# ablab/spades

Hardware: NVIDIA H100
Metric: Mk-mers/s (extract+count+index) k=55, 150 bp reads (higher is better)
Workload: dtype u64

## Files before the change

spades_b200/csrc/count.cu:

```cuda
#include <time.h>

#include <algorithm>

#include "sgpu_internal.h"

namespace sg {

__device__ __forceinline__ void prefetch_l2(const void *p) { asm volatile("prefetch.global.L2 [%0];" ::"l"(p)); }

struct ReadsSrc {
    const uint64_t *words;
    const uint64_t *offs;
    const uint32_t *lens;
    int64_t n;
    uint64_t nwords;
    int K;
    static constexpr int kIds = 24;
    static constexpr int kIdLines = 48;
    static constexpr bool kSubRanges = true;
    __device__ __forceinline__ uint64_t first_word(int64_t item) const { return offs[item]; }
    __device__ __forceinline__ uint32_t len(int64_t item) const { return lens[item]; }
    __device__ __forceinline__ void prefetch_items(int64_t item, int lane) const {
        if (lane == 0) prefetch_l2(lens + item);
        else if (lane == 1 && item + 16 < n) prefetch_l2(offs + item + 16);
// ... 172 lines not shown
    const int lane = threadIdx.x & 31;
    const int64_t item = t * kRollTile + lane;
    uint32_t s = 0;
    if (item < src.n) {
        const int L = (int)src.len(item);
        const uint32_t w = L >= src.K ? (uint32_t)(L - src.K + 1) : 0u;
        s = (w + kRollWin<BOTH> - 1) / kRollWin<BOTH>;
    }
    for (int o = 16; o; o >>= 1) s += __shfl_down_sync(0xffffffffu, s, o);
    if (lane == 0) out[t] = s * Src::kIds;
}

struct RollUnit { int it, j0, cnt; };
template <bool BOTH>
__device__ __forceinline__ RollUnit roll_unit(const RollWarp &rw, int nitems, uint32_t u, uint32_t unif, int K) {
    constexpr int C = kRollWin<BOTH>;
    RollUnit q;
    q.it = find_item_u(rw.pref, nitems, u, unif);
    q.j0 = (int)(u - rw.pref[q.it]) * C;
    const int nwin = (int)rw.len[q.it] - K + 1;
    q.cnt = nwin - q.j0 < C ? nwin - q.j0 : C;
    return q;
}

template <int NW, class Src, bool BOTH>
__global__ void __launch_bounds__(kRollThreads, 2) levelA_count_roll_k(Src src, LevelA p, uint32_t *__restrict__ blk_counts,
                                                                      const uint64_t *__restrict__ tile_off, uint16_t *__restrict__ ids) {
    extern __shared__ __align__(16) unsigned char sm_raw[];
    uint32_t *hist = reinterpret_cast<uint32_t *>(sm_raw);
    RollWarp &rw = *roll_warp_slice(sm_raw, p.PA);
    for (uint32_t i = threadIdx.x; i < p.PA; i += blockDim.x) hist[i] = 0;
    __syncthreads();
    const int K = p.K;
    const int lane = threadIdx.x & 31, warp = threadIdx.x >> 5;
    const int64_t ntiles = (src.n + kRollTile - 1) / kRollTile;
    const int64_t per = (ntiles + gridDim.x - 1) / gridDim.x;
    const int64_t t0 = (int64_t)blockIdx.x * per, t1 = min(ntiles, t0 + per);
    for (int64_t t = t0 + warp; t < t1; t += kRollWarps) {
        const int64_t item0 = t * kRollTile;
        const int nitems = (int)min((int64_t)kRollTile, src.n - item0);
        uint32_t unif = 0;
        bool staged = false;
        const bool has_next = t + kRollWarps < t1;
        const int64_t nx = (t + kRollWarps) * kRollTile;
        uint64_t next_w0 = 0;
        if (has_next) {
            next_w0 = src.first_word(nx);
            src.prefetch_items(nx, lane);
        }
        const uint32_t nunits = roll_warp_setup<BOTH>(src, item0, nitems, rw, &unif, &staged);
        uint64_t *row = ids ? reinterpret_cast<uint64_t *>(ids + tile_off[t]) : nullptr;
        for (uint32_t u = lane; u < nunits; u += 32) {
            const RollUnit q = roll_unit<BOTH>(rw, nitems, u, unif, K);
            const uint64_t *seq = staged ? static_cast<const uint64_t *>(rw.words + rw.off[q.it]) : src.words + src.first_word(item0 + q.it);
            RollState<NW> st;
            roll_init<NW>(st, seq, q.j0, K, q.cnt);
            const int nrec = BOTH ? 2 * q.cnt : q.cnt;
#pragma unroll 1
            for (int g = 0; g < Src::kIds / 4; ++g) {
                uint64_t acc = 0;
#pragma unroll
                for (int e = 0; e < 4; ++e) {
                    const int s = 4 * g + e;
                    uint32_t id = 0xffffu;
                    if (s < nrec) {
                        if (s > 0 && !(BOTH && (e & 1))) roll_next<NW>(st, K);
                        const Kmer<NW> k = BOTH ? ((e & 1) ? st.r : st.f) : kmer_is_minimal<NW>(st.f, st.r) ? st.f : st.r;
                        uint32_t part;
                        if (part_of<NW>(p, k, &part)) { atomicAdd(&hist[part], 1u); id = part; }
                    }
                    acc |= (uint64_t)id << (16 * e);
                }
                if (row) row[(size_t)u * (Src::kIds / 4) + g] = acc;
            }
        }
        if (has_next && lane < 10 && next_w0 + 16 * lane < src.nwords) prefetch_l2(src.words + next_w0 + 16 * lane);
        __syncwarp();
    }
    __syncthreads();
    uint32_t *out = blk_counts + (size_t)blockIdx.x * p.PA;
    for (uint32_t i = threadIdx.x; i < p.PA; i += blockDim.x) out[i] += hist[i];
}

static const uint32_t kABatchNoTag = 0xffffffffu;
static const int kABatchPartBits = 13;
static const uint32_t kABatchMin = 1024;
template <int NW> struct ABatch {
    static constexpr size_t rec_bytes() { return NW * sizeof(uint64_t) + sizeof(uint32_t) + sizeof(uint16_t); }
};
__host__ __device__ __forceinline__ size_t abatch_offset(uint32_t PA) {
    return ((((size_t)2 * PA * 4 + 15) & ~(size_t)15) + (size_t)kRollWarps * sizeof(RollWarp) + 15) & ~(size_t)15;
}

template <int NW, class Src, bool BOTH, bool HAS_IDS>
__global__ void __launch_bounds__(kRollThreads, 2) levelA_scatter_roll_k(Src src, LevelA p, uint64_t *__restrict__ base, uint64_t *__restrict__ out,
                                                                        const uint64_t *__restrict__ tile_off, const uint16_t *__restrict__ ids,
                                                                        uint32_t id_lo, uint32_t row_stride, uint32_t q_lo, uint64_t ids_len, uint32_t cap) {
    extern __shared__ __align__(16) unsigned char sm_raw[];
    __shared__ uint32_t s_fill;
    __shared__ uint32_t warp_tot[kRollWarps];
    const uint32_t PA = p.PA;
    uint32_t *cur = reinterpret_cast<uint32_t *>(sm_raw);
    uint32_t *cnt = cur + PA;
    RollWarp &rw = *roll_warp_slice(sm_raw, 2 * PA);
    uint64_t *stage = reinterpret_cast<uint64_t *>(sm_raw + abatch_offset(PA));
    uint32_t *tags = reinterpret_cast<uint32_t *>(stage + (size_t)cap * NW);
    uint16_t *idx = reinterpret_cast<uint16_t *>(tags + cap);
    uint64_t *mybase = base + (size_t)blockIdx.x * row_stride + q_lo;
    const uint64_t region0 = mybase[0];
    for (uint32_t i = threadIdx.x; i < PA; i += blockDim.x) { cur[i] = (uint32_t)(mybase[i] - region0); cnt[i] = 0; }
    if (threadIdx.x == 0) s_fill = 0;
    __syncthreads();
    uint64_t *const out0 = out + region0 * NW;
    const int K = p.K;
    const int lane = threadIdx.x & 31, warp = threadIdx.x >> 5;
    const uint32_t lt_mask = (1u << lane) - 1u;
    const int64_t ntiles = (src.n + kRollTile - 1) / kRollTile;
    const int64_t per = (ntiles + gridDim.x - 1) / gridDim.x;
    const int64_t t0 = (int64_t)blockIdx.x * per, t1 = min(ntiles, t0 + per);

    int64_t t = t0 + warp;
    bool need_setup = true;
    int nitems = 0;
    uint32_t nunits = 0, unif = 0;
    bool staged = false;
    uint64_t next_w0 = 0, next_row = 0;
    const ulonglong2 *row = nullptr;
    int u = 0, s = 0, cnt_w = 0;
    RollState<NW> st;
    uint64_t idq[Src::kIds / 4];
    for (;;) {
        while (t < t1) {
            if (need_setup) {
                const int64_t item0 = t * kRollTile;
                nitems = (int)min((int64_t)kRollTile, src.n - item0);
                const int64_t nx = (t + kRollWarps) * kRollTile;
                if (t + kRollWarps < t1) {
                    next_w0 = src.first_word(nx);
                    src.prefetch_items(nx, lane);
                    if (HAS_IDS) next_row = tile_off[t + kRollWarps];
                }
                nunits = roll_warp_setup<BOTH>(src, item0, nitems, rw, &unif, &staged);
                if (HAS_IDS) row = reinterpret_cast<const ulonglong2 *>(ids + tile_off[t]);
                u = lane - 32; s = cnt_w = 0;
                need_setup = false;
            }
            if (s >= cnt_w && u < (int)nunits) {
                u += 32;
                if (u < (int)nunits) {
                    if (HAS_IDS) {
#pragma unroll
                        for (int v = 0; v < Src::kIds / 8; ++v) {
                            const ulonglong2 x = __ldg(row + (size_t)u * (Src::kIds / 8) + v);
                            idq[2 * v] = x.x; idq[2 * v + 1] = x.y;
                        }
                    }
                    const RollUnit q = roll_unit<BOTH>(rw, nitems, (uint32_t)u, unif, K);
                    const uint64_t *seq = staged ? static_cast<const uint64_t *>(rw.words + rw.off[q.it]) : src.words + src.first_word(t * kRollTile + q.it);
                    roll_init<NW>(st, seq, q.j0, K, q.cnt);
                    s = 0; cnt_w = BOTH ? 2 * q.cnt : q.cnt;
                }
            }
            const bool act = s < cnt_w;
            if (!__any_sync(0xffffffffu, act)) {
                if (t + kRollWarps < t1) {
                    if (lane < 10 && next_w0 + 16 * lane < src.nwords) prefetch_l2(src.words + next_w0 + 16 * lane);
                    if (HAS_IDS) {
                        if ((Src::kIdLines >= 32 || lane < Src::kIdLines) && next_row + 64 * lane < ids_len) prefetch_l2(ids + next_row + 64 * lane);
                        if (lane < Src::kIdLines - 32 && next_row + 64 * (32 + lane) < ids_len) prefetch_l2(ids + next_row + 64 * (32 + lane));
                    }
                }
                __syncwarp();
                t += kRollWarps;
                need_setup = true;
                continue;
            }
            uint32_t part = 0;
            bool mine = false;
            Kmer<NW> k;
            if (act) {
                if (HAS_IDS) {
                    part = (uint32_t)(idq[0] & 0xffffu) - id_lo;
                    mine = part < PA;
                }
                if (!HAS_IDS || mine) {
                    const bool fwd = BOTH ? !(s & 1) : kmer_is_minimal<NW>(st.f, st.r);
#pragma unroll
                    for (int j = 0; j < NW; ++j) k.w[j] = fwd ? st.f.w[j] : st.r.w[j];
                }
                if (!HAS_IDS) mine = part_of<NW>(p, k, &part);
            }
            const uint32_t bal = __ballot_sync(0xffffffffu, mine);
            if (bal) {
                const uint32_t n = __popc(bal);
                uint32_t b0 = 0;
                if (lane == 0) b0 = atomicAdd(&s_fill, n);
                b0 = __shfl_sync(0xffffffffu, b0, 0);
                if (b0 + n > cap) {
                    if (b0 < cap && (uint32_t)lane < cap - b0) tags[b0 + lane] = kABatchNoTag;
                    break;
                }
                if (mine) {
                    const uint32_t i = b0 + __popc(bal & lt_mask);
                    const uint32_t rank = atomicAdd(&cnt[part], 1u) & 0xffffu;
                    store_rec<NW>(stage + (size_t)i * NW, k);
                    tags[i] = (rank << kABatchPartBits) | part;
                }
            }
            if (act && ++s < cnt_w) {
                if (!BOTH || !(s & 1)) roll_next<NW>(st, K);
                if (HAS_IDS) {
                    if ((s & 3) == 0) {
#pragma unroll
                        for (int v = 0; v + 1 < Src::kIds / 4; ++v) idq[v] = idq[v + 1];
                    } else {
                        idq[0] >>= 16;
                    }
                }
            }
        }
        const bool more = __syncthreads_or(t < t1);
        const uint32_t nslots = min(s_fill, cap);
        const uint32_t own = (PA + kRollThreads - 1) / kRollThreads;
        const uint32_t j0 = min(PA, threadIdx.x * own), j1 = min(PA, j0 + own);
        uint32_t sum = 0;
        for (uint32_t j = j0; j < j1; ++j) sum += cnt[j] & 0xffffu;
        uint32_t inc = sum;
#pragma unroll
        for (int o = 1; o < 32; o <<= 1) {
            const uint32_t v = __shfl_up_sync(0xffffffffu, inc, o);
            if (lane >= o) inc += v;
        }
        if (lane == 31) warp_tot[warp] = inc;
        __syncthreads();
        uint32_t wb = 0, total = 0;
#pragma unroll
        for (int w = 0; w < kRollWarps; ++w) { const uint32_t v = warp_tot[w]; if (w < warp) wb += v; total += v; }
        uint32_t o = wb + inc - sum;
        for (uint32_t j = j0; j < j1; ++j) {
            const uint32_t c = cnt[j] & 0xffffu;
            o += c;
            cnt[j] = o << 16;
            cur[j] += c;
        }
        if (threadIdx.x == 0) s_fill = 0;
        __syncthreads();
        for (uint32_t i = threadIdx.x; i < nslots; i += kRollThreads) {
            const uint32_t tg = tags[i];
            if (tg == kABatchNoTag) continue;
            idx[(cnt[tg & ((1u << kABatchPartBits) - 1)] >> 16) - 1 - (tg >> kABatchPartBits)] = (uint16_t)i;
        }
        __syncthreads();
        for (uint32_t q = threadIdx.x; q < total; q += kRollThreads) {
            const uint32_t i = idx[q], tg = tags[i];
            const uint32_t slot = cur[tg & ((1u << kABatchPartBits) - 1)] - 1 - (tg >> kABatchPartBits);
            store_rec_stream<NW>(out0 + (size_t)slot * NW, load_rec<NW>(stage + (size_t)i * NW));
        }
        __syncthreads();
        if (!more) break;
    }
    for (uint32_t i = threadIdx.x; i < PA; i += blockDim.x) mybase[i] = region0 + cur[i];
}

struct Seg {
    uint64_t start;
    uint64_t len;
    uint32_t bits;
    uint32_t bb;
};

__global__ void seg_init_k(const uint64_t *__restrict__ part_start, const uint64_t *__restrict__ part_total, uint32_t PA, int rA,
                           uint32_t b_lo, Seg *__restrict__ segs) {
    uint32_t part = blockIdx.x * blockDim.x + threadIdx.x;
    if (part >= PA) return;
    Seg s;
    s.start = part_start[part]; s.len = part_total[part]; s.bits = (uint32_t)rA; s.bb = ((b_lo + (part >> rA)) << 1) | 0u;
    segs[part] = s;
}

struct Pieces {
    const uint64_t *pbase;
    const uint32_t *cnt;
    uint32_t cnt_stride, PA;
    int G;
};
static const int kMaxPieces = 1024;

__global__ void stage_rows_k(const uint32_t *__restrict__ cnt, uint32_t cnt_stride, uint32_t PA, uint64_t *__restrict__ rel, uint64_t *__restrict__ row_total) {
    __shared__ uint64_t wsum[8];
    __shared__ uint64_t carry_s;
    const uint32_t *row = cnt + (size_t)blockIdx.x * cnt_stride;
    uint64_t *out = rel + (size_t)blockIdx.x * PA;
    const int lane = threadIdx.x & 31, warp = threadIdx.x >> 5;
    if (threadIdx.x == 0) carry_s = 0;
    __syncthreads();
    for (uint32_t b = 0; b < PA; b += blockDim.x) {
        const uint32_t i = b + threadIdx.x;
        const uint64_t v = i < PA ? row[i] : 0;
        uint64_t inc = v;
#pragma unroll
        for (int o = 1; o < 32; o <<= 1) {
            uint64_t t = __shfl_up_sync(0xffffffffu, inc, o);
            if (lane >= o) inc += t;
        }
        if (lane == 31) wsum[warp] = inc;
        __syncthreads();
        uint64_t wb = 0, all = 0;
        for (int w = 0; w < 8; ++w) { if (w < warp) wb += wsum[w]; all += wsum[w]; }
        const uint64_t carry = carry_s;
        if (i < PA) out[i] = carry + wb + inc - v;
        __syncthreads();
        if (threadIdx.x == 0) carry_s = carry + all;
        __syncthreads();
    }
    if (threadIdx.x == 0) row_total[blockIdx.x] = carry_s;
}
__global__ void stage_add_k(uint64_t *__restrict__ rel, const uint64_t *__restrict__ row_start, uint32_t PA, int G) {
    const uint64_t i = (uint64_t)blockIdx.x * blockDim.x + threadIdx.x;
    if (i >= (uint64_t)G * PA) return;
    rel[i] += row_start[i / PA];
}

struct RefinePlan { uint32_t cap, target, rmax; int total_bits; };
__device__ __forceinline__ int plan_r(const RefinePlan &rp, uint64_t len, uint32_t bits) {
    if (len <= rp.cap) return 0;
    int rem = rp.total_bits - (int)bits;
    if (rem <= 0) return 0;
    uint64_t want = (len + rp.target - 1) / rp.target;
    int r = 1;
    while (r < (int)rp.rmax && (1ull << r) < want) ++r;
    return r < rem ? r : rem;
}
__global__ void refine_plan_k(const Seg *__restrict__ segs, uint64_t n, RefinePlan rp, uint32_t *__restrict__ nchild, uint32_t *__restrict__ isw, int force_all) {
    uint64_t i = (uint64_t)blockIdx.x * blockDim.x + threadIdx.x;
    if (i >= n) return;
    int r = plan_r(rp, segs[i].len, segs[i].bits);
    nchild[i] = r ? (1u << r) : 1u;
    isw[i] = (r || force_all) ? 1u : 0u;
}
__global__ void refine_copy_k(const Seg *__restrict__ segs, uint64_t n, const uint32_t *__restrict__ isw, const uint64_t *__restrict__ child_base,
                              const uint64_t *__restrict__ work_pos, Seg *__restrict__ nsegs, uint64_t *__restrict__ worklist) {
// ... 622 lines not shown
            refine_k<NW, false><<<grid, kRThreads, sm, st>>>(segs.p, worklist.p, tot[1], cbase.p, rp, K, X.p, Y.p, nsegs_arr.p, wcounter.p, Pieces());
        }
        ctx->launches++;
        SG_CUDA(cudaGetLastError());
        tr.mark("refine round");
        (round == 0 ? ctx->times.refine_splits_round0 : ctx->times.refine_splits_later) += tot[0] - nsegs;
        ++rounds;
        segs = std::move(nsegs_arr);
        nsegs = tot[0];
    }
    ctx->times.refine_rounds_max = std::max(ctx->times.refine_rounds_max, rounds);
    ctx->times.refine += tm.stop();
    DArr<uint32_t> ndist(ctx, nsegs + 1);
    DArr<unsigned long long> stats(ctx, 4);
    SG_CUDA(cudaMemsetAsync(ndist.p, 0, ndist.bytes(), st));
    SG_CUDA(cudaMemsetAsync(stats.p, 0, 32, st));
    SG_CUDA(cudaMemsetAsync(wcounter.p, 0, 8, st));
    tm.start();
    {
        auto launch = [&](auto kernel, size_t smem) {
            SG_CUDA(cudaFuncSetAttribute(kernel, cudaFuncAttributeMaxDynamicSharedMemorySize, (int)smem));
            int occ = 1;
            SG_CUDA(cudaOccupancyMaxActiveBlocksPerMultiprocessor(&occ, kernel, kSThreads, smem));
            if (occ < 1) occ = 1;
            int grid = (int)std::min<uint64_t>(nsegs, (uint64_t)ctx->num_sms * occ);
            if (grid < 1) grid = 1;
            kernel<<<grid, kSThreads, smem, st>>>(segs.p, nsegs, K, X.p, Y.p, ndist.p, wcounter.p, stats.p);
        };
        constexpr int bins = 1 << kSortBinBits;
        launch(local_sort3_k<NW, kSortBinBits, CAP>, (size_t)(CAP + kResCap) * NW * sizeof(uint64_t) + (size_t)3 * bins * sizeof(uint32_t) +
                                                         ((size_t)2 * bins + 2 + kResCap) * sizeof(uint16_t) + 16);
        ctx->launches++;
        SG_CUDA(cudaGetLastError());
    }
    DArr<uint64_t> dbase(ctx, nsegs + 1);
    exclusive_scan_u32_to_u64(ctx, ndist.p, dbase.p, nsegs + 1);
    uint64_t D = 0;
    unsigned long long h_stats[4];
    SG_CUDA(cudaMemcpyAsync(&D, dbase.p + nsegs, 8, cudaMemcpyDeviceToHost, st));
    SG_CUDA(cudaMemcpyAsync(h_stats, stats.p, 32, cudaMemcpyDeviceToHost, st));
    SG_CUDA(cudaStreamSynchronize(st));
    ctx->times.local_sort += tm.stop();
    tr.mark("local sort");
    SG_CHECK(h_stats[0] == 0, 6, "internal: oversize segment with unfixed key bits reached the local sort");
    ctx->times.sort_lsd_fallbacks += h_stats[1];
    ctx->times.sort_oversize_equal += h_stats[2];
    Chunk ch;
    ch.n = (int64_t)D; ch.b_lo = (int)b_lo; ch.b_hi = b_hi; ch.first = first;
    ch.keys.alloc(ctx, (size_t)D * NW + 2, true);
    if (want_counts) ch.counts.alloc(ctx, (size_t)D + 1, true);
    tm.start();
    if (nsegs) {
        compact_k<NW><<<div_up((int64_t)nsegs * 32, 256), 256, 0, st>>>(segs.p, nsegs, ndist.p, dbase.p, X.p, Y.p, K, want_counts ? 1 : 0,
                                                                     double_selfrc ? 1 : 0, ch.keys.p, ch.counts.p, d_bsz_p);
        ctx->launches++;
        SG_CUDA(cudaGetLastError());
    }
    ctx->times.compact += tm.stop();
    tr.mark("compact");
    ch_out = std::move(ch);
}

template <int NW, class Src, bool BOTH>
struct LevelAJob {
    Ctx *ctx = nullptr;
    std::vector<Src> srcs;
    int K = 0, B = 0, rA = 0, G = 0;
    int s_lo = 0, s_hi = 0;
    uint32_t PA_all = 0;
    bool use_ids = false;
    DArr<uint32_t> blk_counts;
    DArr<uint64_t> part_total_all;
    std::vector<DArr<uint64_t>> tile_off;
    std::vector<DArr<uint16_t>> ids;
    std::vector<uint64_t> h_part;
    uint64_t bucket_records(int b) const {
        uint64_t s = 0;
        for (uint32_t q = 0; q < (1u << rA); ++q) s += h_part[((size_t)(b - s_lo) << rA) + q];
        return s;
    }
};

static int levelA_ctas_per_sm() { return 2; }
template <int NW>
static size_t levelA_batch_smem(uint32_t PA, uint32_t *cap) {
    static_assert(kLevelAMaxParts <= (1 << kABatchPartBits), "a batch tag holds the partition");
    int dev = 0, per_sm = 0, per_cta = 0, reserved = 0;
    SG_CUDA(cudaGetDevice(&dev));
    SG_CUDA(cudaDeviceGetAttribute(&per_sm, cudaDevAttrMaxSharedMemoryPerMultiprocessor, dev));
    SG_CUDA(cudaDeviceGetAttribute(&per_cta, cudaDevAttrMaxSharedMemoryPerBlockOptin, dev));
    SG_CUDA(cudaDeviceGetAttribute(&reserved, cudaDevAttrReservedSharedMemoryPerBlock, dev));
    const size_t rec = ABatch<NW>::rec_bytes(), fixed = abatch_offset(PA), kStatic = 128;
    size_t room = (size_t)per_sm / levelA_ctas_per_sm() - (size_t)reserved - kStatic;
    if (room < fixed + kABatchMin * rec) room = (size_t)per_cta - kStatic;
    SG_CHECK(room >= fixed + kABatchMin * rec, 6, "internal: level-A batch does not fit shared memory");
    *cap = (uint32_t)std::min<size_t>((room - fixed) / rec, 32768) & ~31u;
    return fixed + (size_t)*cap * rec;
}
static int levelA_key_bits(uint64_t est_records, int B, int total_bits, uint32_t target, uint32_t pa_max) {
    const int want = ilog2_floor(est_records / target + 1) + 1;
    const int bbits = ilog2_floor((uint64_t)B) + (((1u << ilog2_floor((uint64_t)B)) < (uint32_t)B) ? 1 : 0);
    int rA = want - bbits;
    if (rA < 0) rA = 0;
    while (rA > 0 && ((uint64_t)B << rA) > pa_max) --rA;
    if (rA > total_bits) rA = total_bits;
    if (rA > 13) rA = 13;
    return rA;
}

template <int NW, class Src, bool BOTH>
static void levelA_count(LevelAJob<NW, Src, BOTH> &job, Timer &tm, Trace &tr) {
    Ctx *ctx = job.ctx;
    cudaStream_t st = ctx->stream;
    const uint32_t PA_all = job.PA_all;
    const int G = job.G;
    SG_CHECK(PA_all >= 1 && PA_all <= (uint32_t)kLevelAMaxParts, 6, "internal: level-A partition table too large");
    LevelA pa_all;
    pa_all.K = job.K; pa_all.B = (uint32_t)job.B; pa_all.b_lo = (uint32_t)job.s_lo; pa_all.b_hi = (uint32_t)job.s_hi; pa_all.rA = job.rA; pa_all.PA = PA_all;
    job.blk_counts.alloc(ctx, (size_t)G * PA_all);
    job.part_total_all.alloc(ctx, (size_t)PA_all + 1);
    job.h_part.assign(PA_all, 0);
    SG_CUDA(cudaMemsetAsync(job.blk_counts.p, 0, job.blk_counts.bytes(), st));
    job.tile_off.clear(); job.ids.clear();
    job.tile_off.resize(job.srcs.size()); job.ids.resize(job.srcs.size());
    const double free0 = (double)ctx->free_bytes();
    std::vector<uint64_t> nslots(job.srcs.size(), 0);
    uint64_t all_slots = 0;
    for (size_t si = 0; si < job.srcs.size(); ++si) {
        const Src &src = job.srcs[si];
        if (src.n == 0) continue;
        const int64_t ntiles = (src.n + kRollTile - 1) / kRollTile;
        DArr<uint32_t> ttot(ctx, (size_t)ntiles + 1);
        job.tile_off[si].alloc(ctx, (size_t)ntiles + 1);
        SG_CUDA(cudaMemsetAsync(ttot.p + ntiles, 0, 4, st));
        roll_tile_ids_k<BOTH><<<div_up(ntiles, 8), 256, 0, st>>>(src, ntiles, ttot.p);
        ctx->launches++;
        exclusive_scan_u32_to_u64(ctx, ttot.p, job.tile_off[si].p, (size_t)ntiles + 1);
        SG_CUDA(cudaMemcpyAsync(&nslots[si], job.tile_off[si].p + ntiles, 8, cudaMemcpyDeviceToHost, st));
        SG_CUDA(cudaStreamSynchronize(st));
        all_slots += nslots[si];
    }
    job.use_ids = PA_all < 0xffffu && (double)all_slots * 2.0 < free0 * 0.20;
    for (size_t si = 0; si < job.srcs.size(); ++si) {
        if (!job.use_ids) job.tile_off[si] = DArr<uint64_t>();
        else if (job.srcs[si].n) job.ids[si].alloc(ctx, (size_t)nslots[si] + 8);
    }
    tm.start();
    SG_CUDA(cudaFuncSetAttribute(levelA_count_roll_k<NW, Src, BOTH>, cudaFuncAttributeMaxDynamicSharedMemorySize, (int)roll_smem_bytes(PA_all)));
    for (size_t si = 0; si < job.srcs.size(); ++si) {
        const Src &src = job.srcs[si];
        if (src.n == 0) continue;
        levelA_count_roll_k<NW, Src, BOTH><<<G, kRollThreads, roll_smem_bytes(PA_all), st>>>(src, pa_all, job.blk_counts.p, job.tile_off[si].p, job.ids[si].p);
        ctx->launches++;
    }
    SG_CUDA(cudaGetLastError());
    levelA_totals_k<<<div_up(PA_all, 256), 256, 0, st>>>(job.blk_counts.p, PA_all, G, job.part_total_all.p);
    ctx->launches++;
    SG_CUDA(cudaMemcpyAsync(job.h_part.data(), job.part_total_all.p, (size_t)PA_all * 8, cudaMemcpyDeviceToHost, st));
    SG_CUDA(cudaStreamSynchronize(st));
    ctx->times.extract_count += tm.stop();
    tr.mark("A1 count+totals");
}

template <int NW, class Src, bool BOTH>
static void levelA_scatter(LevelAJob<NW, Src, BOTH> &job, int b_lo, int b_hi, uint64_t I_pass, uint64_t total_records, uint64_t *X, uint64_t *pbase_buf,
                           Pieces &pcs, Timer &tm, Trace &tr) {
    Ctx *ctx = job.ctx;
    cudaStream_t st = ctx->stream;
    const int G = job.G;
    const uint32_t PA_all = job.PA_all;
    const uint32_t p_lo = (uint32_t)(b_lo - job.s_lo) << job.rA;
    LevelA pa;
    pa.K = job.K; pa.B = (uint32_t)job.B; pa.b_lo = (uint32_t)b_lo; pa.b_hi = (uint32_t)b_hi; pa.rA = job.rA; pa.PA = (uint32_t)(b_hi - b_lo) << job.rA;
    const uint32_t PA = pa.PA;
    SG_CHECK(PA >= 1 && PA <= (uint32_t)kLevelAMaxParts && G <= kMaxPieces, 6, "internal: level-A pass geometry");
    DArr<uint64_t> base(ctx, (size_t)G * PA);
    {
        DArr<uint64_t> row_total(ctx, (size_t)G + 1), row_start(ctx, (size_t)G + 1);
        SG_CUDA(cudaMemsetAsync(row_total.p + G, 0, 8, st));
        stage_rows_k<<<G, 256, 0, st>>>(job.blk_counts.p + p_lo, PA_all, PA, base.p, row_total.p);
        exclusive_scan_u64(ctx, row_total.p, row_start.p, (size_t)G + 1);
        stage_add_k<<<div_up((int64_t)G * PA, 256), 256, 0, st>>>(base.p, row_start.p, PA, G);
        ctx->launches += 2;
        SG_CUDA(cudaMemcpyAsync(pbase_buf, base.p, (size_t)G * PA * 8, cudaMemcpyDeviceToDevice, st));
    }
    pcs.pbase = pbase_buf; pcs.cnt = job.blk_counts.p + p_lo; pcs.cnt_stride = PA_all; pcs.PA = PA; pcs.G = G;
    tm.start();
    int nsub_auto = (int)(4.0 * (double)I_pass / (double)std::max<uint64_t>(1, total_records) + 0.5);
    nsub_auto = std::min(4, std::max(1, nsub_auto));
    uint32_t nsub = job.use_ids && !BOTH && Src::kSubRanges ? (uint32_t)(tuning().a_sub ? tuning().a_sub : nsub_auto) : 1u;
    if (nsub > PA) nsub = PA;
    for (uint32_t sb = 0; sb < nsub; ++sb) {
        const uint32_t q_lo = (uint32_t)((uint64_t)PA * sb / nsub), q_hi = (uint32_t)((uint64_t)PA * (sb + 1) / nsub);
        if (q_hi == q_lo) continue;
        LevelA pa_sub = pa;
        pa_sub.PA = q_hi - q_lo;
        uint32_t cap = 0;
        const size_t smem = levelA_batch_smem<NW>(pa_sub.PA, &cap);
        if (job.use_ids) SG_CUDA(cudaFuncSetAttribute(levelA_scatter_roll_k<NW, Src, BOTH, true>, cudaFuncAttributeMaxDynamicSharedMemorySize, (int)smem));
        else SG_CUDA(cudaFuncSetAttribute(levelA_scatter_roll_k<NW, Src, BOTH, false>, cudaFuncAttributeMaxDynamicSharedMemorySize, (int)smem));
        for (size_t si = 0; si < job.srcs.size(); ++si) {
            const Src &src = job.srcs[si];
            if (src.n == 0) continue;
            if (job.use_ids)
                levelA_scatter_roll_k<NW, Src, BOTH, true><<<G, kRollThreads, smem, st>>>(src, pa_sub, base.p, X, job.tile_off[si].p, job.ids[si].p, p_lo + q_lo, PA, q_lo, (uint64_t)job.ids[si].n, cap);
            else
                levelA_scatter_roll_k<NW, Src, BOTH, false><<<G, kRollThreads, smem, st>>>(src, pa, base.p, X, nullptr, nullptr, 0u, PA, 0u, 0ull, cap);
            ctx->launches++; ctx->times.level_a_scatters++;
        }
    }
    SG_CUDA(cudaGetLastError());
    ctx->times.extract_scatter += tm.stop();
    tr.mark("A2 scatter");
}

static double pass_bytes_needed(uint64_t recs, size_t W) { return (double)recs * W * 2.0 + (double)recs * (W + 4) * 0.6 + (64 << 20); }

template <int NW, bool BOTH, class Src>
static void run_count(Ctx *ctx, const std::vector<Src> &srcs, int K, int B, bool want_counts, bool double_selfrc, uint64_t est_records, KSet *out) {
    const int total_bits = 2 * K;
    const size_t W = 8 * NW;
    cudaStream_t st = ctx->stream;
    Timer tm(st);
    Trace tr(st);

    out->bsz.assign(B, 0);
    DArr<unsigned long long> d_bsz(ctx, B);
    SG_CUDA(cudaMemsetAsync(d_bsz.p, 0, B * sizeof(unsigned long long), st));

    const int rA = levelA_key_bits(est_records, B, total_bits, sort_target<NW>(), tuning().pa_max);
    ctx->times.level_a_key_bits = (uint64_t)rA;
    const int SR = std::max(1, kLevelAMaxParts >> rA);
    const int n_ranges = (B + SR - 1) / SR;
    int64_t first = 0;
    for (int s_lo = 0; s_lo < B; s_lo += SR) {
        const int share = (kMaxChunks - (int)out->chunks.size()) / (n_ranges - s_lo / SR);
        LevelAJob<NW, Src, BOTH> job;
        job.ctx = ctx; job.srcs = srcs; job.K = K; job.B = B; job.rA = rA; job.G = ctx->num_sms * levelA_ctas_per_sm();
        job.s_lo = s_lo; job.s_hi = std::min(B, s_lo + SR);
        job.PA_all = (uint32_t)(job.s_hi - job.s_lo) << rA;
        levelA_count(job, tm, tr);
        auto current_limit = [&]() {
            return ctx->hbm_budget ? (ctx->hbm_budget > ctx->allocated ? ctx->hbm_budget - ctx->allocated : 0) : (size_t)(ctx->free_bytes() * 0.90);
        };
        uint64_t total_records = 0;
        for (int b = job.s_lo; b < job.s_hi; ++b) total_records += job.bucket_records(b);
        uint64_t pass_target = total_records;
        bool capped = false;
        {
            double lim_sim = (double)current_limit();
            int npass_sim = 0, b = job.s_lo;
            while (b < job.s_hi) {
                uint64_t I = 0; const int b0 = b;
                while (b < job.s_hi) {
                    const uint64_t ib = job.bucket_records(b);
                    if (b > b0 && pass_bytes_needed(I + ib, W) > lim_sim) break;
                    I += ib; ++b;
                }
                lim_sim -= (double)I * (W + 4) * 0.5;
                ++npass_sim;
            }
            capped = npass_sim > share;
            pass_target = total_records / (uint64_t)std::min(npass_sim, share) + total_records / 64 + 1;
        }
        int b_lo = job.s_lo, npass = 0;
        while (b_lo < job.s_hi) {
            const int left = share - npass;
            const int min_b = (capped || left == 1) ? div_up(job.s_hi - b_lo, left) : 1;
            const size_t lim = current_limit();
            int b_hi = b_lo;
            uint64_t I = 0;
            while (b_hi < job.s_hi) {
                const uint64_t ib = job.bucket_records(b_hi);
                if (b_hi - b_lo >= min_b && (pass_bytes_needed(I + ib, W) > (double)lim || I + ib > pass_target)) break;
                I += ib; ++b_hi;
            }
            ++npass;
            const uint32_t p_lo = (uint32_t)(b_lo - job.s_lo) << rA;
            const uint32_t PA = (uint32_t)(b_hi - b_lo) << rA;
            DArr<uint64_t> part_total(ctx, PA + 1), part_start(ctx, PA + 1);
            SG_CUDA(cudaMemcpyAsync(part_total.p, job.part_total_all.p + p_lo, (size_t)PA * 8, cudaMemcpyDeviceToDevice, st));
            SG_CUDA(cudaMemsetAsync(part_total.p + PA, 0, 8, st));
            exclusive_scan_u64(ctx, part_total.p, part_start.p, PA + 1);
            ctx->times.passes++;
            ctx->times.instances += I;
            DArr<uint64_t> X(ctx, (size_t)I * NW + 2), Y(ctx, (size_t)I * NW + 2);
            DArr<uint64_t> pbase(ctx, (size_t)job.G * PA);
            Pieces pcs;
            levelA_scatter(job, b_lo, b_hi, I, total_records, X.p, pbase.p, pcs, tm, tr);
            Chunk ch;
// ... 557 lines not shown
```

Baseline: 8097.

## Add planned level-A scatter kernel that pre-counts partition ids per batch

```diff
diff --git a/spades_b200/csrc/count.cu b/spades_b200/csrc/count.cu
--- a/spades_b200/csrc/count.cu
+++ b/spades_b200/csrc/count.cu
@@ -278,20 +278,19 @@
     for (uint32_t i = threadIdx.x; i < p.PA; i += blockDim.x) out[i] += hist[i];
 }
 
+static const uint32_t kABatchMin = 1024;
+static_assert(kABatchMin / kRollWarps >= 32 * 2, "a warp's share of the smallest batch holds one window of a warp step");
+__host__ __device__ __forceinline__ size_t abatch_offset(uint32_t PA) {
+    return ((((size_t)2 * PA * 4 + 15) & ~(size_t)15) + (size_t)kRollWarps * sizeof(RollWarp) + 15) & ~(size_t)15;
+}
+template <int NW, bool PLANNED>
+constexpr size_t abatch_rec_bytes() { return NW * sizeof(uint64_t) + (PLANNED ? sizeof(uint16_t) : sizeof(uint32_t) + sizeof(uint16_t)); }
+
 static const uint32_t kABatchNoTag = 0xffffffffu;
 static const int kABatchPartBits = 13;
-static const uint32_t kABatchMin = 1024;
-template <int NW> struct ABatch {
-    static constexpr size_t rec_bytes() { return NW * sizeof(uint64_t) + sizeof(uint32_t) + sizeof(uint16_t); }
-};
-__host__ __device__ __forceinline__ size_t abatch_offset(uint32_t PA) {
-    return ((((size_t)2 * PA * 4 + 15) & ~(size_t)15) + (size_t)kRollWarps * sizeof(RollWarp) + 15) & ~(size_t)15;
-}
-
-template <int NW, class Src, bool BOTH, bool HAS_IDS>
+template <int NW, class Src, bool BOTH>
 __global__ void __launch_bounds__(kRollThreads, 2) levelA_scatter_roll_k(Src src, LevelA p, uint64_t *__restrict__ base, uint64_t *__restrict__ out,
-                                                                        const uint64_t *__restrict__ tile_off, const uint16_t *__restrict__ ids,
-                                                                        uint32_t id_lo, uint32_t row_stride, uint32_t q_lo, uint64_t ids_len, uint32_t cap) {
+                                                                        uint32_t row_stride, uint32_t cap) {
     extern __shared__ __align__(16) unsigned char sm_raw[];
     __shared__ uint32_t s_fill;
     __shared__ uint32_t warp_tot[kRollWarps];
@@ -302,7 +301,7 @@
     uint64_t *stage = reinterpret_cast<uint64_t *>(sm_raw + abatch_offset(PA));
     uint32_t *tags = reinterpret_cast<uint32_t *>(stage + (size_t)cap * NW);
     uint16_t *idx = reinterpret_cast<uint16_t *>(tags + cap);
-    uint64_t *mybase = base + (size_t)blockIdx.x * row_stride + q_lo;
+    uint64_t *mybase = base + (size_t)blockIdx.x * row_stride;
     const uint64_t region0 = mybase[0];
     for (uint32_t i = threadIdx.x; i < PA; i += blockDim.x) { cur[i] = (uint32_t)(mybase[i] - region0); cnt[i] = 0; }
     if (threadIdx.x == 0) s_fill = 0;
@@ -320,11 +319,9 @@
     int nitems = 0;
     uint32_t nunits = 0, unif = 0;
     bool staged = false;
-    uint64_t next_w0 = 0, next_row = 0;
-    const ulonglong2 *row = nullptr;
+    uint64_t next_w0 = 0;
     int u = 0, s = 0, cnt_w = 0;
     RollState<NW> st;
-    uint64_t idq[Src::kIds / 4];
     for (;;) {
         while (t < t1) {
             if (need_setup) {
@@ -334,23 +331,14 @@
                 if (t + kRollWarps < t1) {
                     next_w0 = src.first_word(nx);
                     src.prefetch_items(nx, lane);
-                    if (HAS_IDS) next_row = tile_off[t + kRollWarps];
                 }
                 nunits = roll_warp_setup<BOTH>(src, item0, nitems, rw, &unif, &staged);
-                if (HAS_IDS) row = reinterpret_cast<const ulonglong2 *>(ids + tile_off[t]);
                 u = lane - 32; s = cnt_w = 0;
                 need_setup = false;
             }
             if (s >= cnt_w && u < (int)nunits) {
                 u += 32;
                 if (u < (int)nunits) {
-                    if (HAS_IDS) {
-#pragma unroll
-                        for (int v = 0; v < Src::kIds / 8; ++v) {
-                            const ulonglong2 x = __ldg(row + (size_t)u * (Src::kIds / 8) + v);
-                            idq[2 * v] = x.x; idq[2 * v + 1] = x.y;
-                        }
-                    }
                     const RollUnit q = roll_unit<BOTH>(rw, nitems, (uint32_t)u, unif, K);
                     const uint64_t *seq = staged ? static_cast<const uint64_t *>(rw.words + rw.off[q.it]) : src.words + src.first_word(t * kRollTile + q.it);
                     roll_init<NW>(st, seq, q.j0, K, q.cnt);
@@ -359,13 +347,7 @@
             }
             const bool act = s < cnt_w;
             if (!__any_sync(0xffffffffu, act)) {
-                if (t + kRollWarps < t1) {
-                    if (lane < 10 && next_w0 + 16 * lane < src.nwords) prefetch_l2(src.words + next_w0 + 16 * lane);
-                    if (HAS_IDS) {
-                        if ((Src::kIdLines >= 32 || lane < Src::kIdLines) && next_row + 64 * lane < ids_len) prefetch_l2(ids + next_row + 64 * lane);
-                        if (lane < Src::kIdLines - 32 && next_row + 64 * (32 + lane) < ids_len) prefetch_l2(ids + next_row + 64 * (32 + lane));
-                    }
-                }
+                if (t + kRollWarps < t1 && lane < 10 && next_w0 + 16 * lane < src.nwords) prefetch_l2(src.words + next_w0 + 16 * lane);
                 __syncwarp();
                 t += kRollWarps;
                 need_setup = true;
@@ -375,16 +357,10 @@
             bool mine = false;
             Kmer<NW> k;
             if (act) {
-                if (HAS_IDS) {
-                    part = (uint32_t)(idq[0] & 0xffffu) - id_lo;
-                    mine = part < PA;
-                }
-                if (!HAS_IDS || mine) {
-                    const bool fwd = BOTH ? !(s & 1) : kmer_is_minimal<NW>(st.f, st.r);
-#pragma unroll
-                    for (int j = 0; j < NW; ++j) k.w[j] = fwd ? st.f.w[j] : st.r.w[j];
-                }
-                if (!HAS_IDS) mine = part_of<NW>(p, k, &part);
+                const bool fwd = BOTH ? !(s & 1) : kmer_is_minimal<NW>(st.f, st.r);
+#pragma unroll
+                for (int j = 0; j < NW; ++j) k.w[j] = fwd ? st.f.w[j] : st.r.w[j];
+                mine = part_of<NW>(p, k, &part);
             }
             const uint32_t bal = __ballot_sync(0xffffffffu, mine);
             if (bal) {
@@ -403,17 +379,7 @@
                     tags[i] = (rank << kABatchPartBits) | part;
                 }
             }
-            if (act && ++s < cnt_w) {
-                if (!BOTH || !(s & 1)) roll_next<NW>(st, K);
-                if (HAS_IDS) {
-                    if ((s & 3) == 0) {
-#pragma unroll
-                        for (int v = 0; v + 1 < Src::kIds / 4; ++v) idq[v] = idq[v + 1];
-                    } else {
-                        idq[0] >>= 16;
-                    }
-                }
-            }
+            if (act && ++s < cnt_w && (!BOTH || !(s & 1))) roll_next<NW>(st, K);
         }
         const bool more = __syncthreads_or(t < t1);
         const uint32_t nslots = min(s_fill, cap);
@@ -453,6 +419,191 @@
             store_rec_stream<NW>(out0 + (size_t)slot * NW, load_rec<NW>(stage + (size_t)i * NW));
         }
         __syncthreads();
+        if (!more) break;
+    }
+    for (uint32_t i = threadIdx.x; i < PA; i += blockDim.x) mybase[i] = region0 + cur[i];
+}
+
+template <int NW, class Src, bool BOTH>
+__global__ void __launch_bounds__(kRollThreads, 2) levelA_scatter_plan_k(Src src, LevelA p, uint64_t *__restrict__ base, uint64_t *__restrict__ out,
+                                                                        const uint64_t *__restrict__ tile_off, const uint16_t *__restrict__ ids,
+                                                                        uint32_t id_lo, uint32_t row_stride, uint32_t q_lo, uint64_t ids_len, uint32_t cap) {
+    extern __shared__ __align__(16) unsigned char sm_raw[];
+    __shared__ uint32_t warp_tot[kRollWarps];
+    constexpr int kR = BOTH ? 2 : 1;
+    constexpr int kRowV = Src::kIds / 8;
+    const uint32_t PA = p.PA;
+    uint32_t *cur = reinterpret_cast<uint32_t *>(sm_raw);
+    uint32_t *run = cur + PA;
+    RollWarp &rw = *roll_warp_slice(sm_raw, 2 * PA);
+    uint64_t *stage = reinterpret_cast<uint64_t *>(sm_raw + abatch_offset(PA));
+    uint16_t *ptag = reinterpret_cast<uint16_t *>(stage + (size_t)cap * NW);
+    uint64_t *mybase = base + (size_t)blockIdx.x * row_stride + q_lo;
+    const uint64_t region0 = mybase[0];
+    for (uint32_t i = threadIdx.x; i < PA; i += blockDim.x) { cur[i] = (uint32_t)(mybase[i] - region0); run[i] = 0; }
+    __syncthreads();
+    uint64_t *const out0 = out + region0 * NW;
+    const int K = p.K;
+    const int lane = threadIdx.x & 31, warp = threadIdx.x >> 5;
+    const int64_t ntiles = (src.n + kRollTile - 1) / kRollTile;
+    const int64_t per = (ntiles + gridDim.x - 1) / gridDim.x;
+    const int64_t t0 = (int64_t)blockIdx.x * per, t1 = min(ntiles, t0 + per);
+    const uint32_t share = cap / kRollWarps;
+
+    int64_t pt = t0 + warp;
+    int pj = 0, ps = 0;
+    uint32_t pn = 0;
+    bool p_enter = true;
+    const ulonglong2 *prow = nullptr;
+    int64_t rt = pt;
+    int rj = 0, rs = 0;
+    bool need_setup = true;
+    int nitems = 0;
+    uint32_t nunits = 0, unif = 0;
+    bool staged = false;
+    uint64_t next_w0 = 0;
+    const ulonglong2 *row = nullptr;
+    for (;;) {
+        uint32_t room = share;
+        while (pt < t1) {
+            if (p_enter) {
+                const uint64_t a = tile_off[pt], b = tile_off[pt + 1];
+                if (pt + kRollWarps < t1) {
+                    const uint64_t nr = tile_off[pt + kRollWarps];
+                    if ((Src::kIdLines >= 32 || lane < Src::kIdLines) && nr + 64 * lane < ids_len) prefetch_l2(ids + nr + 64 * lane);
+                    if (lane < Src::kIdLines - 32 && nr + 64 * (32 + lane) < ids_len) prefetch_l2(ids + nr + 64 * (32 + lane));
+                }
+                pn = (uint32_t)((b - a) / Src::kIds);
+                prow = reinterpret_cast<const ulonglong2 *>(ids + a);
+                p_enter = false;
+            }
+            if ((uint32_t)pj * 32 >= pn) {
+                pt += kRollWarps; pj = 0; ps = 0; p_enter = true;
+                continue;
+            }
+            if (room < 32 * kR) break;
+            const uint32_t u = (uint32_t)pj * 32 + lane;
+            uint64_t idq[Src::kIds / 4];
+#pragma unroll
+            for (int v = 0; v < kRowV; ++v) {
+                ulonglong2 x = make_ulonglong2(~0ull, ~0ull);
+                if (u < pn) x = __ldg(prow + (size_t)u * kRowV + v);
+                idq[2 * v] = x.x; idq[2 * v + 1] = x.y;
+            }
+            int end = Src::kIds;
+#pragma unroll
+            for (int e = 0; e < Src::kIds; e += kR) {
+                uint32_t part[kR];
+                bool own[kR];
+                uint32_t c = 0;
+#pragma unroll
+                for (int r = 0; r < kR; ++r) {
+                    part[r] = (uint32_t)((idq[(e + r) / 4] >> (16 * ((e + r) % 4))) & 0xffffu) - id_lo;
+                    own[r] = e >= ps && part[r] < PA;
+                    c += __popc(__ballot_sync(0xffffffffu, own[r]));
+                }
+                if (c > room) { end = e; break; }
+                room -= c;
+#pragma unroll
+                for (int r = 0; r < kR; ++r) if (own[r]) atomicAdd(&run[part[r]], 1u);
+            }
+            if (end < Src::kIds) { ps = end; break; }
+            ++pj; ps = 0;
+        }
+        const bool more = __syncthreads_or(pt < t1);
+        const uint32_t own = (PA + kRollThreads - 1) / kRollThreads;
+        const uint32_t j0 = min(PA, threadIdx.x * own), j1 = min(PA, j0 + own);
+        uint32_t sum = 0;
+        for (uint32_t j = j0; j < j1; ++j) sum += run[j] & 0xffffu;
+        uint32_t inc = sum;
+#pragma unroll
+        for (int o = 1; o < 32; o <<= 1) {
+            const uint32_t v = __shfl_up_sync(0xffffffffu, inc, o);
+            if (lane >= o) inc += v;
+        }
+        if (lane == 31) warp_tot[warp] = inc;
+        __syncthreads();
+        uint32_t wb = 0, total = 0;
+#pragma unroll
+        for (int w = 0; w < kRollWarps; ++w) { const uint32_t v = warp_tot[w]; if (w < warp) wb += v; total += v; }
+        uint32_t o = wb + inc - sum;
+        for (uint32_t j = j0; j < j1; ++j) {
+            const uint32_t c = run[j] & 0xffffu;
+            run[j] = o << 16;
+            o += c;
+            cur[j] += c;
+        }
+        __syncthreads();
+        while (rt < pt || (rt == pt && (rj < pj || (rj == pj && rs < ps)))) {
+            if (need_setup) {
+                const int64_t item0 = rt * kRollTile;
+                nitems = (int)min((int64_t)kRollTile, src.n - item0);
+                const int64_t nx = (rt + kRollWarps) * kRollTile;
+                if (rt + kRollWarps < t1) {
+                    next_w0 = src.first_word(nx);
+                    src.prefetch_items(nx, lane);
+                }
+                nunits = roll_warp_setup<BOTH>(src, item0, nitems, rw, &unif, &staged);
+                row = reinterpret_cast<const ulonglong2 *>(ids + tile_off[rt]);
+                need_setup = false;
+            }
+            if ((uint32_t)rj * 32 >= nunits) {
+                if (rt + kRollWarps < t1 && lane < 10 && next_w0 + 16 * lane < src.nwords) prefetch_l2(src.words + next_w0 + 16 * lane);
+                __syncwarp();
+                rt += kRollWarps; rj = 0; rs = 0;
+                need_setup = true;
+                continue;
+            }
+            const int end = (rt == pt && rj == pj) ? ps : Src::kIds;
+            const int u = rj * 32 + lane;
+            if (u < (int)nunits) {
+                const RollUnit q = roll_unit<BOTH>(rw, nitems, (uint32_t)u, unif, K);
+                const int s_end = min(end, BOTH ? 2 * q.cnt : q.cnt);
+                if (rs < s_end) {
+                    uint64_t idq[Src::kIds / 4];
+#pragma unroll
+                    for (int v = 0; v < kRowV; ++v) {
+                        const ulonglong2 x = __ldg(row + (size_t)u * kRowV + v);
+                        idq[2 * v] = x.x; idq[2 * v + 1] = x.y;
+                    }
+                    for (int w = 0; w < rs / 4; ++w) {
+#pragma unroll
+                        for (int v = 0; v + 1 < Src::kIds / 4; ++v) idq[v] = idq[v + 1];
+                    }
+                    idq[0] >>= 16 * (rs & 3);
+                    const uint64_t *seq = staged ? static_cast<const uint64_t *>(rw.words + rw.off[q.it]) : src.words + src.first_word(rt * kRollTile + q.it);
+                    RollState<NW> st;
+                    roll_init<NW>(st, seq, q.j0 + rs / kR, K, q.cnt - rs / kR);
+                    for (int s = rs;;) {
+                        const uint32_t part = (uint32_t)(idq[0] & 0xffffu) - id_lo;
+                        if (part < PA) {
+                            const bool fwd = BOTH ? !(s & 1) : kmer_is_minimal<NW>(st.f, st.r);
+                            Kmer<NW> k;
+#pragma unroll
+                            for (int j = 0; j < NW; ++j) k.w[j] = fwd ? st.f.w[j] : st.r.w[j];
+                            const uint32_t pos = atomicAdd(&run[part], 1u << 16) >> 16;
+                            store_rec<NW>(stage + (size_t)pos * NW, k);
+                            ptag[pos] = (uint16_t)part;
+                        }
+                        if (++s >= s_end) break;
+                        if (!BOTH || !(s & 1)) roll_next<NW>(st, K);
+                        if ((s & 3) == 0) {
+#pragma unroll
+                            for (int v = 0; v + 1 < Src::kIds / 4; ++v) idq[v] = idq[v + 1];
+                        } else {
+                            idq[0] >>= 16;
+                        }
+                    }
+                }
+            }
+            if (end == Src::kIds) { ++rj; rs = 0; } else rs = end;
+        }
+        __syncthreads();
+        for (uint32_t q = threadIdx.x; q < total; q += kRollThreads) {
+            const uint32_t part = ptag[q];
+            const uint32_t slot = cur[part] - (run[part] >> 16) + q;
+            store_rec_stream<NW>(out0 + (size_t)slot * NW, load_rec<NW>(stage + (size_t)q * NW));
+        }
         if (!more) break;
     }
     for (uint32_t i = threadIdx.x; i < PA; i += blockDim.x) mybase[i] = region0 + cur[i];
@@ -1241,19 +1392,20 @@
 };
 
 static int levelA_ctas_per_sm() { return 2; }
-template <int NW>
+template <int NW, bool PLANNED>
 static size_t levelA_batch_smem(uint32_t PA, uint32_t *cap) {
-    static_assert(kLevelAMaxParts <= (1 << kABatchPartBits), "a batch tag holds the partition");
+    static_assert(kLevelAMaxParts <= (1 << kABatchPartBits) && kLevelAMaxParts <= 0xffff, "a batch tag holds the partition");
     int dev = 0, per_sm = 0, per_cta = 0, reserved = 0;
     SG_CUDA(cudaGetDevice(&dev));
     SG_CUDA(cudaDeviceGetAttribute(&per_sm, cudaDevAttrMaxSharedMemoryPerMultiprocessor, dev));
     SG_CUDA(cudaDeviceGetAttribute(&per_cta, cudaDevAttrMaxSharedMemoryPerBlockOptin, dev));
     SG_CUDA(cudaDeviceGetAttribute(&reserved, cudaDevAttrReservedSharedMemoryPerBlock, dev));
-    const size_t rec = ABatch<NW>::rec_bytes(), fixed = abatch_offset(PA), kStatic = 128;
+    const size_t rec = abatch_rec_bytes<NW, PLANNED>(), fixed = abatch_offset(PA), kStatic = 128;
     size_t room = (size_t)per_sm / levelA_ctas_per_sm() - (size_t)reserved - kStatic;
     if (room < fixed + kABatchMin * rec) room = (size_t)per_cta - kStatic;
     SG_CHECK(room >= fixed + kABatchMin * rec, 6, "internal: level-A batch does not fit shared memory");
     *cap = (uint32_t)std::min<size_t>((room - fixed) / rec, 32768) & ~31u;
+    SG_CHECK(!PLANNED || *cap / kRollWarps >= 32 * 2, 6, "internal: level-A warp share below one window step");
     return fixed + (size_t)*cap * rec;
 }
 static int levelA_key_bits(uint64_t est_records, int B, int total_bits, uint32_t target, uint32_t pa_max) {
@@ -1355,16 +1507,16 @@
         LevelA pa_sub = pa;
         pa_sub.PA = q_hi - q_lo;
         uint32_t cap = 0;
-        const size_t smem = levelA_batch_smem<NW>(pa_sub.PA, &cap);
-        if (job.use_ids) SG_CUDA(cudaFuncSetAttribute(levelA_scatter_roll_k<NW, Src, BOTH, true>, cudaFuncAttributeMaxDynamicSharedMemorySize, (int)smem));
-        else SG_CUDA(cudaFuncSetAttribute(levelA_scatter_roll_k<NW, Src, BOTH, false>, cudaFuncAttributeMaxDynamicSharedMemorySize, (int)smem));
+        const size_t smem = job.use_ids ? levelA_batch_smem<NW, true>(pa_sub.PA, &cap) : levelA_batch_smem<NW, false>(pa_sub.PA, &cap);
+        if (job.use_ids) SG_CUDA(cudaFuncSetAttribute(levelA_scatter_plan_k<NW, Src, BOTH>, cudaFuncAttributeMaxDynamicSharedMemorySize, (int)smem));
+        else SG_CUDA(cudaFuncSetAttribute(levelA_scatter_roll_k<NW, Src, BOTH>, cudaFuncAttributeMaxDynamicSharedMemorySize, (int)smem));
         for (size_t si = 0; si < job.srcs.size(); ++si) {
             const Src &src = job.srcs[si];
             if (src.n == 0) continue;
             if (job.use_ids)
-                levelA_scatter_roll_k<NW, Src, BOTH, true><<<G, kRollThreads, smem, st>>>(src, pa_sub, base.p, X, job.tile_off[si].p, job.ids[si].p, p_lo + q_lo, PA, q_lo, (uint64_t)job.ids[si].n, cap);
+                levelA_scatter_plan_k<NW, Src, BOTH><<<G, kRollThreads, smem, st>>>(src, pa_sub, base.p, X, job.tile_off[si].p, job.ids[si].p, p_lo + q_lo, PA, q_lo, (uint64_t)job.ids[si].n, cap);
             else
-                levelA_scatter_roll_k<NW, Src, BOTH, false><<<G, kRollThreads, smem, st>>>(src, pa, base.p, X, nullptr, nullptr, 0u, PA, 0u, 0ull, cap);
+                levelA_scatter_roll_k<NW, Src, BOTH><<<G, kRollThreads, smem, st>>>(src, pa, base.p, X, PA, cap);
             ctx->launches++; ctx->times.level_a_scatters++;
         }
     }
```

New measurement: 8366 (median of 6 runs). 3.3% higher.
